# SYNCC-IN/hyperscanning-signal-analysis

Hardware: AMD Instinct MI355X
Metric: MVAR+ffDTF windows/sec, 2x32-ch dyad p=8, 256 freqs (higher is better)
Workload: dtype f64; 1 GPU; C2: 1 dyad(s)/GPU, 2x32 ch @500 Hz, 10 min, 2 s windows 50% overlap (599 windows per dyad), MVAR p=8, 256 freqs 0.5-128 Hz; dyads_per_gpu=1, k1=hop blocks summed once, shared by the overlapping windows (hop 500), k2=block Levinson-Whittle recursion, one workgroup per window, one launch, normalisation=inside K3 (rows of window w by workgroups of window w+lag), parallelism=dyad-sharded x1, gather=none

## Files before the change

hyperscanning_signal_analysis_amd/csrc/lagcov.hip:

```cpp
#include "hmv_common.h"
#include "hmv_kernels.h"
#include <cstdlib>

namespace hmv {

constexpr int LC_TC = 64;
constexpr int LC_HALO = 32;
constexpr int LC_S = LC_TC + LC_HALO + 6;

template <int NT, int LG>
__global__ void __launch_bounds__(256, 2) lagcov_kernel(LagcovArgs a) {
  constexpr int MP = 16 * NT, NIW = NT, NJ = NT;
  __shared__ double xs[MP * LC_S];
  const int l = lane_id();
  const int wv = uni(threadIdx.x >> 6);
  const long long item = blockIdx.x;
  const int lag0 = blockIdx.y * LG;
  const int nl = min(LG, a.p + 1 - lag0);
  const int i = l >> 4, cc = l & 15;
  const int n = a.n, m = a.m;
  const bool blk = a.blocks != 0;
  const long long start = blk ? a.blk_first + item * (long long)n : a.item_start[item];
  const double* x = a.x + (blk ? 0 : a.item_rec[item] * a.rec_stride) + start;
  const long long vlen = blk ? a.blk_T - start : (long long)n;
  const bool mask_a = blk && (n & 3) != 0;

  double acc[LG][NIW][NJ];
#pragma unroll
  for (int g = 0; g < LG; ++g)
#pragma unroll
    for (int I = 0; I < NIW; ++I)
#pragma unroll
      for (int J = 0; J < NJ; ++J) acc[g][I][J] = 0.0;

  constexpr int W = LC_TC + LC_HALO;
  constexpr int NLD = (MP * W + 255) / 256;
  for (int t0 = 0; t0 < n; t0 += LC_TC) {
    double stg[NLD];
#pragma unroll
    for (int r = 0; r < NLD; ++r) {
      const int idx = threadIdx.x + 256 * r;
      const int ch = idx / W, tt = idx - ch * W;
      const int t = t0 + tt;
      stg[r] = (idx < MP * W && ch < m && t < vlen) ? x[(size_t)ch * a.ld + t] : 0.0;
    }
    __syncthreads();
#pragma unroll
    for (int r = 0; r < NLD; ++r) {
      const int idx = threadIdx.x + 256 * r;
      const int ch = idx / W, tt = idx - ch * W;
      if (idx < MP * W) xs[ch * LC_S + tt] = stg[r];
    }
    __syncthreads();
    const int steps = min(LC_TC, n - t0 + 3) >> 2;
    const double* xa = xs + (4 * NT * wv + (l & 3)) * LC_S + (l >> 4);
    const double* xb = xs + cc * LC_S + lag0 + (l >> 4);
    for (int ts = 0; ts < steps; ++ts) {
      double av[NIW];
#pragma unroll
      for (int I = 0; I < NIW; ++I) av[I] = xa[4 * I * LC_S + 4 * ts];
      if (mask_a && t0 + 4 * ts + 3 >= n) {
        const bool in = t0 + 4 * ts + (l >> 4) < n;
#pragma unroll
        for (int I = 0; I < NIW; ++I) av[I] = in ? av[I] : 0.0;
      }
      static_for<LG>([&](auto gc) __attribute__((always_inline)) {
        constexpr int g = decltype(gc)::value;
        if (g < nl) {
          double bv[NJ];
#pragma unroll
          for (int J = 0; J < NJ; ++J) bv[J] = xb[16 * J * LC_S + 4 * ts + g];
#pragma unroll
          for (int I = 0; I < NIW; ++I)
#pragma unroll
            for (int J = 0; J < NJ; ++J) acc[g][I][J] = mfma4(av[I], bv[J], acc[g][I][J]);
        }
      });
    }
  }
  const double scale = blk ? 1.0 : 1.0 / (double)n;
  static_for<LG>([&](auto gc) __attribute__((always_inline)) {
    constexpr int g = decltype(gc)::value;
    if (g < nl) {
      const int lag = lag0 + g;
      double* R = a.R + ((size_t)item * (a.p + 1) + lag) * MP * MP;
#pragma unroll
      for (int I = 0; I < NIW; ++I)
#pragma unroll
        for (int J = 0; J < NJ; ++J) {
          const int row = 4 * (NT * wv + I) + i, col = 16 * J + cc;
          double v = acc[g][I][J] * scale;
          if (!blk && lag == 0 && row == col && row >= m) v = 1.0;
          R[(size_t)row * MP + col] = v;
        }
    }
  });
}

template <int NT>
__global__ void __launch_bounds__(256) lagcomb_kernel(LagcombArgs a) {
  constexpr int MP = 16 * NT, TILE = MP * MP;
  __shared__ double xa[MP * 32], xb[MP * 32];
  const long long w = blockIdx.x;
  const int lag = blockIdx.y;
  const int n = (int)(a.hop * a.k), m = a.m;
  const long long s = a.first + w * a.hop;
  for (int idx = threadIdx.x; idx < MP * lag; idx += 256) {
    const int ch = idx / lag, u = idx - ch * lag;
    const long long ta = s + n - lag + u, tb = s + n + u;
    xa[ch * 32 + u] = (ch < m && ta < a.T) ? a.x[(size_t)ch * a.ld + ta] : 0.0;
    xb[ch * 32 + u] = (ch < m && tb < a.T) ? a.x[(size_t)ch * a.ld + tb] : 0.0;
  }
  __syncthreads();
  const double inv_n = 1.0 / (double)n;
  const double* Q = a.Q + ((size_t)w * (a.p + 1) + lag) * TILE;
  double* R = a.R + ((size_t)w * (a.p + 1) + lag) * TILE;
  for (int e = threadIdx.x; e < TILE; e += 256) {
    const int row = e / MP, col = e - row * MP;
    double acc = 0.0;
    for (int j = 0; j < a.k; ++j) acc += Q[(size_t)j * (a.p + 1) * TILE + e];
    double c = 0.0;
    for (int u = 0; u < lag; ++u) c = __builtin_fma(xa[row * 32 + u], xb[col * 32 + u], c);
    double v = (acc - c) * inv_n;
    if (lag == 0 && row == col && row >= m) v = 1.0;
    R[e] = v;
  }
}

int launch_lagcomb(const LagcombArgs& a, int m_pad, hipStream_t st) {
  if (a.n_win == 0) return 0;
  if (a.p > LC_HALO) return -2;
  const dim3 grid((unsigned)a.n_win, a.p + 1), block(256);
  switch (m_pad) {
    case 16: hipLaunchKernelGGL(lagcomb_kernel<1>, grid, block, 0, st, a); break;
    case 32: hipLaunchKernelGGL(lagcomb_kernel<2>, grid, block, 0, st, a); break;
    case 48: hipLaunchKernelGGL(lagcomb_kernel<3>, grid, block, 0, st, a); break;
    case 64: hipLaunchKernelGGL(lagcomb_kernel<4>, grid, block, 0, st, a); break;
    default: return -1;
  }
  return (int)hipGetLastError();
}

template <int LG>
static int launch_lagcov_lg(const LagcovArgs& a, int m_pad, hipStream_t st) {
  const dim3 grid((unsigned)a.n_items, (a.p + LG) / LG), block(256);
  switch (m_pad) {
    case 16: hipLaunchKernelGGL((lagcov_kernel<1, LG>), grid, block, 0, st, a); break;
    case 32: hipLaunchKernelGGL((lagcov_kernel<2, LG>), grid, block, 0, st, a); break;
    case 48: hipLaunchKernelGGL((lagcov_kernel<3, LG>), grid, block, 0, st, a); break;
    case 64: hipLaunchKernelGGL((lagcov_kernel<4, LG>), grid, block, 0, st, a); break;
    default: return -1;
  }
  return (int)hipGetLastError();
}

int launch_lagcov(const LagcovArgs& a, int m_pad, hipStream_t st) {
  if (a.n_items == 0) return 0;
  if (a.p > LC_HALO) return -2;
  const long long lg = tuning(2 );
  switch (lg) {
    case 1: return launch_lagcov_lg<1>(a, m_pad, st);
    case 2: return launch_lagcov_lg<2>(a, m_pad, st);
    default: return launch_lagcov_lg<3>(a, m_pad, st);
  }
}

}
```

hyperscanning_signal_analysis_amd/csrc/yw_lwr_core.h:

```cpp
#pragma once
#include "yw_common.h"

namespace hmv {

#ifndef HMV_LWR_GUARD
#define HMV_LWR_GUARD 1e-7
#endif

template <int NT, bool VQ, bool AUTO>
__device__ __forceinline__ void yw_lwr_body(const YwArgs& a, const YwAutoArgs& sel) {
  static_assert(VQ || !AUTO, "the selecting form needs every log det Vf_q");
  constexpr int MP = 16 * NT, KH = MP / 2, SH = KH + 6, NIW = NT, NJ = NT, TILE = MP * MP;
  constexpr int NV = (MP * KH / 2 + 255) / 256;
  constexpr int SI = YwCfg<NT>::S;
  constexpr int GEMM_D = 2 * MP * SH, INV_D = MP * SI, BUF_D = GEMM_D > INV_D ? GEMM_D : INV_D;
  __shared__ __attribute__((aligned(16))) double buf[BUF_D];
  __shared__ double Pb[2 * MP * 4];
  __shared__ double Nb[4 * MP * 4];
  __shared__ int s_info;
  __shared__ double s_ld[4];
  __shared__ double s_pm[4 + 4 * 4];
  __shared__ int s_guard;
  __shared__ double s_logdet, s_best;
  __shared__ int s_qstar, s_take;
  double* Xh = buf;
  double* Yh = buf + MP * SH;
  const int wv = uni(threadIdx.x >> 6);
  const int p = a.p;
  const long long item = blockIdx.x;
  double* ws = a.ws + (size_t)item * yw_ws_tiles_d(p) * TILE;
  double* Agen[2] = {ws, ws + (size_t)p * TILE};
  double* Bgen[2] = {ws + (size_t)2 * p * TILE, ws + (size_t)3 * p * TILE};
  double* Vf = ws + (size_t)4 * p * TILE;
  double* Vb = Vf + TILE;
  double* VfI = Vb + TILE;
  double* VbI = VfI + TILE;
  double* Dq = VbI + TILE;
  const double* R = a.R + (size_t)item * (p + 1) * TILE;
  if (threadIdx.x == 0) {
    s_info = 0;
    s_guard = 0;
    if (AUTO) {
      s_best = __builtin_inf();
      s_qstar = 0;
    }
  }

  auto lane = [&]() __attribute__((always_inline)) {
    int lo;
    asm volatile("v_mbcnt_lo_u32_b32 %0, -1, 0\n\tv_mbcnt_hi_u32_b32 %0, -1, %0" : "=v"(lo));
    return lo;
  };
  auto zero = [&](double (&v)[NIW][NJ]) __attribute__((always_inline)) {
#pragma unroll
    for (int ii = 0; ii < NIW; ++ii)
#pragma unroll
      for (int J = 0; J < NJ; ++J) v[ii][J] = 0.0;
  };
  auto fetch = [&](f64x2 (&v)[NV], const double* src, int kh, bool tr) __attribute__((always_inline)) {
    const int t0 = lane() + 64 * wv;
#pragma unroll
    for (int r = 0; r < NV; ++r) {
      const int idx = t0 + 256 * r;
      if (NV * 256 == MP * KH / 2 || idx < MP * KH / 2) {
        if (!tr) {
          const int row = idx / (KH / 2), c2 = idx - row * (KH / 2);
          v[r] = *reinterpret_cast<const f64x2*>(src + (size_t)row * MP + kh * KH + 2 * c2);
        } else {
          const int k = idx / (MP / 2), c2 = idx - k * (MP / 2);
          v[r] = *reinterpret_cast<const f64x2*>(src + (size_t)(kh * KH + k) * MP + 2 * c2);
        }
      }
    }
  };
  auto park = [&](double* dst, const f64x2 (&v)[NV], bool tr) __attribute__((always_inline)) {
    const int t0 = lane() + 64 * wv;
#pragma unroll
    for (int r = 0; r < NV; ++r) {
      const int idx = t0 + 256 * r;
      if (NV * 256 == MP * KH / 2 || idx < MP * KH / 2) {
        if (!tr) {
          const int row = idx / (KH / 2), c2 = idx - row * (KH / 2);
          double* d = dst + row * SH + 2 * c2;
          d[0] = v[r].x;
          d[1] = v[r].y;
        } else {
          const int k = idx / (MP / 2), c2 = idx - k * (MP / 2);
          dst[(2 * c2) * SH + k] = v[r].x;
          dst[(2 * c2 + 1) * SH + k] = v[r].y;
        }
      }
    }
  };
  auto park_strip = [&](const double (&v)[NIW][NJ], int kh) __attribute__((always_inline)) {
    const int l = lane(), i = l >> 4, cc = l & 15;
#pragma unroll
    for (int ii = 0; ii < NIW; ++ii)
#pragma unroll
      for (int J = 0; J < NJ; ++J) {
        const int col = 16 * J + cc - kh * KH;
        if (col >= 0 && col < KH) Xh[(4 * (wv * NT + ii) + i) * SH + col] = v[ii][J];
      }
  };
#ifndef HMV_LWR_GEMM_PIPE
#define HMV_LWR_GEMM_PIPE 1
#endif
  auto gemm_half = [&](double (&acc)[NIW][NJ]) __attribute__((always_inline)) {
    const int l = lane();
    const double* xa = Xh + (4 * wv * NT + (l & 3)) * SH + (l >> 4);
    const double* yb = Yh + (l & 15) * SH + (l >> 4);
#if HMV_LWR_GEMM_PIPE
    constexpr int NS = KH / 4;
    double av[2][NIW], bv[2][NJ];
    auto rd = [&](int set, int k0) __attribute__((always_inline)) {
#pragma unroll
      for (int ii = 0; ii < NIW; ++ii) av[set][ii] = xa[4 * ii * SH + k0];
#pragma unroll
      for (int J = 0; J < NJ; ++J) bv[set][J] = yb[16 * J * SH + k0];
    };
    rd(0, 0);
    static_for<NS>([&](auto sc) __attribute__((always_inline)) {
      constexpr int s = decltype(sc)::value, cur = s & 1;
      if constexpr (s + 1 < NS) rd(cur ^ 1, 4 * (s + 1));
      __builtin_amdgcn_sched_barrier(0);
#pragma unroll
      for (int ii = 0; ii < NIW; ++ii)
#pragma unroll
        for (int J = 0; J < NJ; ++J) acc[ii][J] = mfma4(av[cur][ii], bv[cur][J], acc[ii][J]);
      __builtin_amdgcn_sched_barrier(0);
    });
#else
#pragma unroll 2
    for (int k0 = 0; k0 < KH; k0 += 4) {
      double av[NIW], bv[NJ];
#pragma unroll
      for (int ii = 0; ii < NIW; ++ii) av[ii] = xa[4 * ii * SH + k0];
#pragma unroll
      for (int J = 0; J < NJ; ++J) bv[J] = yb[16 * J * SH + k0];
#pragma unroll
      for (int ii = 0; ii < NIW; ++ii)
#pragma unroll
        for (int J = 0; J < NJ; ++J) acc[ii][J] = mfma4(av[ii], bv[J], acc[ii][J]);
    }
#endif
  };
  auto product = [&](double (&acc)[NIW][NJ], const double* srcX, bool trX, const double (&xr)[NIW][NJ], const double* srcY,
                     bool trY) __attribute__((always_inline)) {
    f64x2 vx[NV], vy[NV];
    if (srcX) fetch(vx, srcX, 0, trX);
    fetch(vy, srcY, 0, trY);
    __syncthreads();
    if (srcX) park(Xh, vx, trX); else park_strip(xr, 0);
    park(Yh, vy, trY);
    if (srcX) fetch(vx, srcX, 1, trX);
    fetch(vy, srcY, 1, trY);
    __syncthreads();
    gemm_half(acc);
    __syncthreads();
    if (srcX) park(Xh, vx, trX); else park_strip(xr, 1);
    park(Yh, vy, trY);
    __syncthreads();
    gemm_half(acc);
  };
  auto store_tile = [&](double* dst, const double (&v)[NIW][NJ]) __attribute__((always_inline)) {
    const int l = lane(), i = l >> 4, cc = l & 15;
#pragma unroll
    for (int ii = 0; ii < NIW; ++ii)
#pragma unroll
      for (int J = 0; J < NJ; ++J) dst[(size_t)(4 * (wv * NT + ii) + i) * MP + 16 * J + cc] = v[ii][J];
  };
  auto load_tile = [&](double (&v)[NIW][NJ], const double* src, bool tr) __attribute__((always_inline)) {
    const int l = lane(), i = l >> 4, cc = l & 15;
#pragma unroll
    for (int ii = 0; ii < NIW; ++ii)
#pragma unroll
      for (int J = 0; J < NJ; ++J) {
        const int row = 4 * (wv * NT + ii) + i, col = 16 * J + cc;
        v[ii][J] = tr ? src[(size_t)col * MP + row] : src[(size_t)row * MP + col];
      }
  };
  auto sub = [&](double (&g)[NIW][NJ], const double (&acc)[NIW][NJ]) __attribute__((always_inline)) {
#pragma unroll
    for (int ii = 0; ii < NIW; ++ii)
#pragma unroll
      for (int J = 0; J < NJ; ++J) g[ii][J] -= acc[ii][J];
  };
  auto invert = [&](const double (&g)[NIW][NJ], double* out, double* logdet, int q) __attribute__((always_inline)) {
    const int info_base = q * MP;
    const int l = lane(), i = l >> 4, cc = l & 15;
    __syncthreads();
#pragma unroll
    for (int ii = 0; ii < NIW; ++ii)
#pragma unroll
      for (int J = 0; J < NJ; ++J) buf[(4 * (wv * NT + ii) + i) * SI + 16 * J + cc] = g[ii][J];
    __syncthreads();
    spd_inverse_coop<NT, SI>(buf, Pb, Nb, &s_info, s_ld, out, logdet, info_base, s_pm);
    if (threadIdx.x == 0 && !(s_pm[0] >= HMV_LWR_GUARD * s_pm[1])) {
      if (!AUTO) s_guard = 1;
      else if (s_guard == 0) s_guard = q + 1;
    }
    __syncthreads();
  };

  auto invert2 = [&](const double (&ga)[NIW][NJ], const double (&gb)[NIW][NJ], double* out_a, double* out_b, double* logdet_b,
                     int q) __attribute__((always_inline)) {
    const int info_base = q * MP;
    spd_inverse_coop2<NT, SI>(ga, gb, buf, Pb, Nb, &s_info, s_ld, out_a, out_b, logdet_b, info_base, s_pm);
    if (threadIdx.x == 0 && (!(s_pm[0] >= HMV_LWR_GUARD * s_pm[1]) || !(s_pm[2] >= HMV_LWR_GUARD * s_pm[3]))) {
      if (!AUTO) s_guard = 1;
      else if (s_guard == 0) s_guard = q + 1;
    }
    __syncthreads();
  };

  auto ld_dst = [&](int q) __attribute__((always_inline)) -> double* {
    if (AUTO) return &s_logdet;
    return a.Vq_logdet + (size_t)item * p + (q - 1);
  };
  auto select = [&](int q) __attribute__((always_inline)) {
    if (threadIdx.x == 0) {
      const double ld = s_logdet;
      const double crit = ld + ((sel.crit_c * (double)q) * (double)(a.m * a.m)) / (double)sel.n;
      if (sel.crit_out) sel.crit_out[(size_t)item * p + (q - 1)] = crit;
      if (a.Vq_logdet) a.Vq_logdet[(size_t)item * p + (q - 1)] = ld;
      const int take = (crit < s_best) ? 1 : 0;
      if (take) {
        s_best = crit;
        s_qstar = q;
      }
      s_take = take;
    }
    __syncthreads();
    if (s_take) {
      const double* Aq = Agen[q & 1];
      double* ar = a.ar + (size_t)item * TILE * p;
      const int total = TILE * q;
      for (int idx = threadIdx.x; idx < total; idx += 256) {
        const int e = idx / q, k = idx - e * q;
        ar[(size_t)e * p + k] = Aq[(size_t)k * TILE + e];
      }
      double* Vo = a.V + (size_t)item * TILE;
      for (int idx = threadIdx.x; idx < TILE; idx += 256) Vo[idx] = Vf[idx];
    }
  };

  double g[NIW][NJ], acc[NIW][NJ], dacc[NIW][NJ];
  const double (&none)[NIW][NJ] = g;
  load_tile(g, R, false);
  store_tile(Vf, g);
  store_tile(Vb, g);
  load_tile(g, R + TILE, true);
  store_tile(Dq, g);
  __syncthreads();
  for (int q = 0; q < p; ++q) {
    const double* Ao = Agen[q & 1];
    const double* Bo = Bgen[q & 1];
    double* An = Agen[(q + 1) & 1];
    double* Bn = Bgen[(q + 1) & 1];
    const bool last = (q == p - 1);
    load_tile(g, Vb, false);
#ifndef HMV_LWR_SINGLE_INVERSES
    if (!last || (VQ && q >= 1)) {
      load_tile(acc, Vf, false);
      invert2(g, acc, VbI, VfI, (VQ && q >= 1) ? ld_dst(q) : nullptr, q);
    } else {
      invert(g, VbI, nullptr, q);
    }
#else
    invert(g, VbI, nullptr, q);
    if (!last || (VQ && q >= 1)) {
      load_tile(g, Vf, false);
      invert(g, VfI, (VQ && q >= 1) ? ld_dst(q) : nullptr, q);
    }
#endif
    if (AUTO && q >= 1) select(q);
    zero(acc);
    product(acc, Dq, false, none, VbI, false);
    store_tile(An + (size_t)q * TILE, acc);
    zero(dacc);
    product(dacc, nullptr, false, acc, Dq, false);
    load_tile(g, Vf, false);
    sub(g, dacc);
    store_tile(Vf, g);
    if (!last) {
      zero(acc);
      product(acc, Dq, true, none, VfI, false);
      store_tile(Bn + (size_t)q * TILE, acc);
      zero(dacc);
      product(dacc, nullptr, false, acc, Dq, true);
      load_tile(g, Vb, false);
      sub(g, dacc);
      store_tile(Vb, g);
    }
    __syncthreads();
    zero(dacc);
    for (int k = 0; k < q; ++k) {
      zero(acc);
      product(acc, An + (size_t)q * TILE, false, none, Bo + (size_t)(q - 1 - k) * TILE, true);
      load_tile(g, Ao + (size_t)k * TILE, false);
      sub(g, acc);
      store_tile(An + (size_t)k * TILE, g);
      if (!last) {
        product(dacc, nullptr, false, g, R + (size_t)(q + 1 - k) * TILE, false);
        zero(acc);
        product(acc, Bn + (size_t)q * TILE, false, none, Ao + (size_t)(q - 1 - k) * TILE, true);
        load_tile(g, Bo + (size_t)k * TILE, false);
        sub(g, acc);
        store_tile(Bn + (size_t)k * TILE, g);
      }
    }
    if (!last) {
      product(dacc, An + (size_t)q * TILE, false, none, R + TILE, false);
      load_tile(g, R + (size_t)(q + 2) * TILE, true);
      sub(g, dacc);
      store_tile(Dq, g);
    }
    __syncthreads();
  }
  if (VQ) {
    load_tile(g, Vf, false);
    invert(g, VfI, ld_dst(p), p);
  }
  if (AUTO) {
    select(p);
    __syncthreads();
    const int bad = s_info, qs = bad ? 0 : s_qstar;
    if (threadIdx.x == 0) {
      a.info[item] = bad ? bad : (qs == 0 ? -1 : 0);
      sel.order_out[item] = qs;
      *yw_guard_ptr(a.ws, item, p, TILE) = (bad == 0 && qs > 0 && s_guard != 0 && s_guard - 1 <= qs) ? 1 : 0;
    }
    double* ar = a.ar + (size_t)item * TILE * p;
    const int total = TILE * p;
    for (int idx = threadIdx.x; idx < total; idx += 256) {
      const int e = idx / p, k = idx - e * p;
      if (k >= qs) ar[idx] = 0.0;
    }
    if (qs == 0) {
      double* Vo = a.V + (size_t)item * TILE;
      for (int idx = threadIdx.x; idx < TILE; idx += 256) Vo[idx] = R[idx];
    }
    return;
  }
  load_tile(g, Vf, false);
  store_tile(a.V + (size_t)item * TILE, g);
  if (threadIdx.x == 0) {
    a.info[item] = s_info;
    *yw_guard_ptr(a.ws, item, p, TILE) = (s_info == 0) ? s_guard : 0;
  }
  const double* Af = Agen[p & 1];
  double* ar = a.ar + (size_t)item * TILE * p;
  const int total = TILE * p;
  for (int idx = threadIdx.x; idx < total; idx += 256) {
    const int e = idx / p, k = idx - e * p;
    ar[idx] = Af[(size_t)k * TILE + e];
  }
}

}
```

Measured before the change: 58720 windows/s.

## Restructure lag-combine staging and cut address arithmetic in block Levinson kernel

The lag-combine kernel now stages one contiguous 2*lag sample strip per channel with wave-coalesced loads, and processes several tile elements per thread so the Q partial-sum loads and lag corrections interleave. The Levinson kernel replaces per-element integer division in fetch, park, load/store tile and the AR-coefficient emit loops with incremental indices. It also uses scalar-base plus small-immediate global addressing via inline asm, aiming to cut VALU address overhead and 64-bit pointer math. The inline asm and address-space casts add fragility and make correctness depend on offset folding.

```diff
diff --git a/hyperscanning_signal_analysis_amd/csrc/lagcov.hip b/hyperscanning_signal_analysis_amd/csrc/lagcov.hip
--- a/hyperscanning_signal_analysis_amd/csrc/lagcov.hip
+++ b/hyperscanning_signal_analysis_amd/csrc/lagcov.hip
@@ -97,33 +97,61 @@
   });
 }
 
+constexpr int LC_CS = 2 * LC_HALO + 1;
 template <int NT>
 __global__ void __launch_bounds__(256) lagcomb_kernel(LagcombArgs a) {
-  constexpr int MP = 16 * NT, TILE = MP * MP;
-  __shared__ double xa[MP * 32], xb[MP * 32];
+  constexpr int MP = 16 * NT, TILE = MP * MP, NE = TILE / 256;
+  constexpr int LC_E = (NE % 4 == 0) ? 4 : (NE % 3 == 0) ? 3 : 1;
+  __shared__ double xs[MP * LC_CS];
   const long long w = blockIdx.x;
   const int lag = blockIdx.y;
   const int n = (int)(a.hop * a.k), m = a.m;
   const long long s = a.first + w * a.hop;
-  for (int idx = threadIdx.x; idx < MP * lag; idx += 256) {
-    const int ch = idx / lag, u = idx - ch * lag;
-    const long long ta = s + n - lag + u, tb = s + n + u;
-    xa[ch * 32 + u] = (ch < m && ta < a.T) ? a.x[(size_t)ch * a.ld + ta] : 0.0;
-    xb[ch * 32 + u] = (ch < m && tb < a.T) ? a.x[(size_t)ch * a.ld + tb] : 0.0;
+  {
+    const int v = threadIdx.x & 63, wv = uni(threadIdx.x >> 6);
+    const long long t = s + n - lag + v;
+    const bool staged = v < 2 * lag, in = staged && t < a.T;
+    const double* xt = a.x + t;
+#pragma unroll
+    for (int j = 0; j < MP / 4; ++j) {
+      const int ch = 4 * j + wv;
+      double val = 0.0;
+      if (in && ch < m) val = xt[(size_t)ch * a.ld];
+      if (staged) xs[ch * LC_CS + v] = val;
+    }
   }
   __syncthreads();
   const double inv_n = 1.0 / (double)n;
+  const size_t qstep = (size_t)(a.p + 1) * TILE;
   const double* Q = a.Q + ((size_t)w * (a.p + 1) + lag) * TILE;
   double* R = a.R + ((size_t)w * (a.p + 1) + lag) * TILE;
-  for (int e = threadIdx.x; e < TILE; e += 256) {
-    const int row = e / MP, col = e - row * MP;
-    double acc = 0.0;
-    for (int j = 0; j < a.k; ++j) acc += Q[(size_t)j * (a.p + 1) * TILE + e];
-    double c = 0.0;
-    for (int u = 0; u < lag; ++u) c = __builtin_fma(xa[row * 32 + u], xb[col * 32 + u], c);
-    double v = (acc - c) * inv_n;
-    if (lag == 0 && row == col && row >= m) v = 1.0;
-    R[e] = v;
+  const int k = a.k;
+  for (int eb = 0; eb < NE; eb += LC_E) {
+    double acc[LC_E], c[LC_E];
+    const double *xa[LC_E], *xb[LC_E];
+#pragma unroll
+    for (int r = 0; r < LC_E; ++r) {
+      const unsigned e = threadIdx.x + 256u * (eb + r), row = e / MP, col = e % MP;
+      xa[r] = xs + row * LC_CS;
+      xb[r] = xs + col * LC_CS + lag;
+      acc[r] = 0.0;
+      c[r] = 0.0;
+    }
+    for (int j = 0; j < k; ++j) {
+#pragma unroll
+      for (int r = 0; r < LC_E; ++r) acc[r] += Q[(size_t)j * qstep + threadIdx.x + 256u * (eb + r)];
+    }
+    for (int u = 0; u < lag; ++u) {
+#pragma unroll
+      for (int r = 0; r < LC_E; ++r) c[r] = __builtin_fma(xa[r][u], xb[r][u], c[r]);
+    }
+#pragma unroll
+    for (int r = 0; r < LC_E; ++r) {
+      const unsigned e = threadIdx.x + 256u * (eb + r), row = e / MP, col = e % MP;
+      double v = (acc[r] - c[r]) * inv_n;
+      if (lag == 0 && row == col && (int)row >= m) v = 1.0;
+      R[e] = v;
+    }
   }
 }
 
diff --git a/hyperscanning_signal_analysis_amd/csrc/yw_lwr_core.h b/hyperscanning_signal_analysis_amd/csrc/yw_lwr_core.h
--- a/hyperscanning_signal_analysis_amd/csrc/yw_lwr_core.h
+++ b/hyperscanning_signal_analysis_amd/csrc/yw_lwr_core.h
@@ -57,58 +57,80 @@
 #pragma unroll
       for (int J = 0; J < NJ; ++J) v[ii][J] = 0.0;
   };
+  auto tid = [&]() __attribute__((always_inline)) {
+    unsigned t;
+    asm volatile("v_mov_b32 %0, %1" : "=v"(t) : "v"(threadIdx.x));
+    return t;
+  };
+  typedef const char __attribute__((address_space(1))) * gcptr;
+  auto gptr = [&](const double* base, unsigned cbytes, unsigned off) __attribute__((always_inline)) {
+    unsigned long long sb = reinterpret_cast<unsigned long long>(base) + (cbytes & ~0xfffu);
+    if (cbytes & ~0xfffu) asm volatile("" : "+s"(sb));
+    return reinterpret_cast<gcptr>(sb) + (cbytes & 0xfffu) + (size_t)off;
+  };
+  constexpr unsigned PR = KH / 2, PT = MP / 2;
+  constexpr bool RSTEP = (256 % PR == 0) && (256 % PT == 0);
   auto fetch = [&](f64x2 (&v)[NV], const double* src, int kh, bool tr) __attribute__((always_inline)) {
-    const int t0 = lane() + 64 * wv;
+    const unsigned t = tid();
+    if (RSTEP) {
+      const unsigned off = !tr ? ((t / PR) * MP + 2 * (t % PR)) * 8u : ((t / PT) * MP + 2 * (t % PT)) * 8u;
+#pragma unroll
+      for (int r = 0; r < NV; ++r) {
+        const unsigned cb = !tr ? (r * (256 / PR) * MP + kh * KH) * 8u : (kh * KH + r * (256 / PT)) * MP * 8u;
+        if (NV * 256 == MP * KH / 2 || t + 256 * r < MP * KH / 2) v[r] = *reinterpret_cast<const f64x2 __attribute__((address_space(1)))*>(gptr(src, cb, off));
+      }
+    } else {
+#pragma unroll
+      for (int r = 0; r < NV; ++r) {
+        const unsigned idx = t + 256 * r;
+        if (NV * 256 == MP * KH / 2 || idx < MP * KH / 2) {
+          const unsigned off = !tr ? ((idx / PR) * MP + 2 * (idx % PR)) * 8u : ((idx / PT) * MP + 2 * (idx % PT)) * 8u;
+          const unsigned cb = !tr ? kh * KH * 8u : kh * KH * MP * 8u;
+          v[r] = *reinterpret_cast<const f64x2 __attribute__((address_space(1)))*>(gptr(src, cb, off));
+        }
+      }
+    }
+  };
+  auto park = [&](double* dst, const f64x2 (&v)[NV], bool tr) __attribute__((always_inline)) {
+    const unsigned t = tid();
 #pragma unroll
     for (int r = 0; r < NV; ++r) {
-      const int idx = t0 + 256 * r;
-      if (NV * 256 == MP * KH / 2 || idx < MP * KH / 2) {
+      const unsigned idx = RSTEP ? t : t + 256 * r;
+      if (NV * 256 == MP * KH / 2 || t + 256 * r < MP * KH / 2) {
         if (!tr) {
-          const int row = idx / (KH / 2), c2 = idx - row * (KH / 2);
-          v[r] = *reinterpret_cast<const f64x2*>(src + (size_t)row * MP + kh * KH + 2 * c2);
-        } else {
-          const int k = idx / (MP / 2), c2 = idx - k * (MP / 2);
-          v[r] = *reinterpret_cast<const f64x2*>(src + (size_t)(kh * KH + k) * MP + 2 * c2);
-        }
-      }
-    }
-  };
-  auto park = [&](double* dst, const f64x2 (&v)[NV], bool tr) __attribute__((always_inline)) {
-    const int t0 = lane() + 64 * wv;
-#pragma unroll
-    for (int r = 0; r < NV; ++r) {
-      const int idx = t0 + 256 * r;
-      if (NV * 256 == MP * KH / 2 || idx < MP * KH / 2) {
-        if (!tr) {
-          const int row = idx / (KH / 2), c2 = idx - row * (KH / 2);
-          double* d = dst + row * SH + 2 * c2;
+          double* d = dst + (RSTEP ? r * (256 / PR) * SH : 0) + ((idx / PR) * SH + 2 * (idx % PR));
           d[0] = v[r].x;
           d[1] = v[r].y;
         } else {
-          const int k = idx / (MP / 2), c2 = idx - k * (MP / 2);
-          dst[(2 * c2) * SH + k] = v[r].x;
-          dst[(2 * c2 + 1) * SH + k] = v[r].y;
+          double* d = dst + (RSTEP ? r * (256 / PT) : 0) + ((2 * (idx % PT)) * SH + idx / PT);
+          d[0] = v[r].x;
+          d[SH] = v[r].y;
         }
       }
     }
   };
   auto park_strip = [&](const double (&v)[NIW][NJ], int kh) __attribute__((always_inline)) {
-    const int l = lane(), i = l >> 4, cc = l & 15;
+    const unsigned l = lane(), i = l >> 4, cc = l & 15;
+    double* d = Xh + (unsigned)(4 * wv * NT) * SH + (i * SH + cc);
 #pragma unroll
     for (int ii = 0; ii < NIW; ++ii)
 #pragma unroll
       for (int J = 0; J < NJ; ++J) {
-        const int col = 16 * J + cc - kh * KH;
-        if (col >= 0 && col < KH) Xh[(4 * (wv * NT + ii) + i) * SH + col] = v[ii][J];
+        const int c0 = 16 * J - kh * KH;
+        if (c0 >= 0 && c0 + 15 < KH) d[4 * ii * SH + c0] = v[ii][J];
+        else if (c0 + 15 >= 0 && c0 < KH) {
+          const int col = c0 + (int)cc;
+          if (col >= 0 && col < KH) d[4 * ii * SH + c0] = v[ii][J];
+        }
       }
   };
 #ifndef HMV_LWR_GEMM_PIPE
 #define HMV_LWR_GEMM_PIPE 1
 #endif
   auto gemm_half = [&](double (&acc)[NIW][NJ]) __attribute__((always_inline)) {
-    const int l = lane();
-    const double* xa = Xh + (4 * wv * NT + (l & 3)) * SH + (l >> 4);
-    const double* yb = Yh + (l & 15) * SH + (l >> 4);
+    const unsigned l = lane();
+    const double* xa = Xh + (unsigned)(4 * wv * NT) * SH + ((l & 3) * SH + (l >> 4));
+    const double* yb = Yh + ((l & 15) * SH + (l >> 4));
 #if HMV_LWR_GEMM_PIPE
     constexpr int NS = KH / 4;
     double av[2][NIW], bv[2][NJ];
@@ -163,20 +185,23 @@
     gemm_half(acc);
   };
   auto store_tile = [&](double* dst, const double (&v)[NIW][NJ]) __attribute__((always_inline)) {
-    const int l = lane(), i = l >> 4, cc = l & 15;
-#pragma unroll
-    for (int ii = 0; ii < NIW; ++ii)
-#pragma unroll
-      for (int J = 0; J < NJ; ++J) dst[(size_t)(4 * (wv * NT + ii) + i) * MP + 16 * J + cc] = v[ii][J];
+    const unsigned l = lane(), off = ((l >> 4) * MP + (l & 15)) * 8u;
+    const double* strip = dst + (unsigned)(4 * wv * NT) * MP;
+#pragma unroll
+    for (int ii = 0; ii < NIW; ++ii)
+#pragma unroll
+      for (int J = 0; J < NJ; ++J)
+        *(double __attribute__((address_space(1)))*)(gptr(strip, (4 * ii * MP + 16 * J) * 8u, off)) = v[ii][J];
   };
   auto load_tile = [&](double (&v)[NIW][NJ], const double* src, bool tr) __attribute__((always_inline)) {
-    const int l = lane(), i = l >> 4, cc = l & 15;
+    const unsigned l = lane(), off = !tr ? ((l >> 4) * MP + (l & 15)) * 8u : ((l & 15) * MP + (l >> 4)) * 8u;
+    const double* strip = src + (unsigned)(4 * wv * NT) * (!tr ? MP : 1);
 #pragma unroll
     for (int ii = 0; ii < NIW; ++ii)
 #pragma unroll
       for (int J = 0; J < NJ; ++J) {
-        const int row = 4 * (wv * NT + ii) + i, col = 16 * J + cc;
-        v[ii][J] = tr ? src[(size_t)col * MP + row] : src[(size_t)row * MP + col];
+        const unsigned cb = !tr ? (4 * ii * MP + 16 * J) * 8u : (16 * J * MP + 4 * ii) * 8u;
+        v[ii][J] = *reinterpret_cast<const double __attribute__((address_space(1)))*>(gptr(strip, cb, off));
       }
   };
   auto sub = [&](double (&g)[NIW][NJ], const double (&acc)[NIW][NJ]) __attribute__((always_inline)) {
@@ -216,6 +241,20 @@
   auto ld_dst = [&](int q) __attribute__((always_inline)) -> double* {
     if (AUTO) return &s_logdet;
     return a.Vq_logdet + (size_t)item * p + (q - 1);
+  };
+  auto emit = [&](const double* Aq, int q) __attribute__((always_inline)) {
+    double* ar = a.ar + (size_t)item * TILE * p;
+    const int total = TILE * q, de = 256 / q, dk = 256 - de * q;
+    int e = (int)threadIdx.x / q, k = (int)threadIdx.x - e * q;
+    for (int idx = threadIdx.x; idx < total; idx += 256) {
+      ar[(size_t)e * p + k] = Aq[(size_t)k * TILE + e];
+      e += de;
+      k += dk;
+      if (k >= q) {
+        k -= q;
+        ++e;
+      }
+    }
   };
   auto select = [&](int q) __attribute__((always_inline)) {
     if (threadIdx.x == 0) {
@@ -232,13 +271,7 @@
     }
     __syncthreads();
     if (s_take) {
-      const double* Aq = Agen[q & 1];
-      double* ar = a.ar + (size_t)item * TILE * p;
-      const int total = TILE * q;
-      for (int idx = threadIdx.x; idx < total; idx += 256) {
-        const int e = idx / q, k = idx - e * q;
-        ar[(size_t)e * p + k] = Aq[(size_t)k * TILE + e];
-      }
+      emit(Agen[q & 1], q);
       double* Vo = a.V + (size_t)item * TILE;
       for (int idx = threadIdx.x; idx < TILE; idx += 256) Vo[idx] = Vf[idx];
     }
@@ -331,10 +364,12 @@
       *yw_guard_ptr(a.ws, item, p, TILE) = (bad == 0 && qs > 0 && s_guard != 0 && s_guard - 1 <= qs) ? 1 : 0;
     }
     double* ar = a.ar + (size_t)item * TILE * p;
-    const int total = TILE * p;
+    const int total = TILE * p, dk = 256 % p;
+    int k = (int)threadIdx.x % p;
     for (int idx = threadIdx.x; idx < total; idx += 256) {
-      const int e = idx / p, k = idx - e * p;
       if (k >= qs) ar[idx] = 0.0;
+      k += dk;
+      k = (k >= p) ? k - p : k;
     }
     if (qs == 0) {
       double* Vo = a.V + (size_t)item * TILE;
@@ -348,13 +383,7 @@
     a.info[item] = s_info;
     *yw_guard_ptr(a.ws, item, p, TILE) = (s_info == 0) ? s_guard : 0;
   }
-  const double* Af = Agen[p & 1];
-  double* ar = a.ar + (size_t)item * TILE * p;
-  const int total = TILE * p;
-  for (int idx = threadIdx.x; idx < total; idx += 256) {
-    const int e = idx / p, k = idx - e * p;
-    ar[idx] = Af[(size_t)k * TILE + e];
-  }
+  emit(Agen[p & 1], p);
 }
 
 }
```

Result: faster. 60310 windows/s (median of 6 runs) (+2.7%).
